# HaokunChen245/FedDAT

Hardware: AMD Instinct MI355X
Metric: VQA samples/sec, ViLT-B/32 dual-adapter local step (higher is better)
Workload: dtype fp16; 1 GPU; configs[1] with fp16 operands (BASELINE.json's configs[1] string says bf16: same operand width and MFMA rate; the bf16 step is in other_operand_format with --full): ViLT-B/32 FedDAT, 1 client per MI355X, fp16 MFMA operands (dynamic loss scale, GradScaler semantics on the device, initial 2^14), fp32 accumulate / masters, batch=32/client, 384x384 synthetic + 40-token questions, MKD on; batch_per_client=32, seq_len=185, clients=1, hip_graph=True, ranks=1, hetero_steps=False

## Files before the change

feddat_amd/albef_engine.py:

```python
from __future__ import annotations

from typing import Dict, List, Optional, Sequence

import torch

from . import lib as L
from .local_update import FlatGroup, LocalUpdateEngine, _bound

PRE = "albef_model.albef."
ADAPTER_TENSORS = ("down.weight", "down.bias", "up.weight", "up.bias")


class AlbefDatEngine(LocalUpdateEngine):
    def __init__(self, params: Dict[str, torch.Tensor], device, batch: int, n_answers: int, q_len: int = 25, a_len: int = 4,
                 vit_depth: int = 12, enc_layers: int = 12, fusion_layer: int = 6, dec_layers: int = 6, image: int = 384,
                 vocab: int = 30522, lr: float = 1e-4, weight_decay: float = 1e-2, adam_eps: float = 1e-8, pad_id: int = 0,
                 max_pos: int = 512, dropout: float = 0.0, seed: int = 0, stack_text: bool = False,
                 operands: str = "f16", loss_scale: Optional[float] = None, dynamic_loss_scale: Optional[bool] = None,
                 scale_growth_interval: int = 2000):
        self._init_loss_scale(operands, loss_scale, dynamic_loss_scale, scale_growth_interval)
        with L.operands(operands):
            self._init(params, device, batch, n_answers, q_len, a_len, vit_depth, enc_layers, fusion_layer, dec_layers, image, vocab,
                       lr, weight_decay, adam_eps, pad_id, max_pos, dropout, seed, stack_text)

# ... 256 lines not shown

    def _wgrad(self, m: int, mode: str, x, dy, rows: int):
        if mode == "both":
            n, h, g = self.ad_numel, rows // 2, self.gs["both"]
            segs = self._wgrad_desc(("wg2", m, x.data_ptr(), dy.data_ptr(), rows), lambda: [
                dict(x=x, dy=dy, z=g["z"], dz=g["dz"], grad=self.ad[0].g[m * n:(m + 1) * n], rows=h, scale=0.5),
                dict(x=x[h:], dy=dy[h:], z=g["z"][h:], dz=g["dz"][h:], grad=self.ad[1].g[m * n:(m + 1) * n], rows=h, scale=1.0)])
            ws = self.wpart_stride2
            L.adapter_wgrad_partial(segs, self.wpart["both"][m * ws:(m + 1) * ws])
            self._wg_done["both"].append(m)
            return
        a = 0 if mode == "gating" else int(mode.split("_")[1])
        if a not in self.opt_adapters:
            return
        n = self.ad_numel
        segs = self._wgrad_desc(("wg", m, a, x.data_ptr(), dy.data_ptr(), rows), lambda: [
            dict(x=x, dy=dy, z=self.gs[mode]["z"], dz=self.gs[mode]["dz"], grad=self.ad[a].g[m * n:(m + 1) * n], rows=rows,
                 scale=0.5 if mode == "gating" else 1.0)])
        ws = self.wpart_stride
        L.adapter_wgrad_partial(segs, self.wpart[mode][m * ws:(m + 1) * ws])
        self._wg_done[mode].append(m)

    def _wgrad_reduce(self, mode: str):
        done, self._wg_done[mode] = self._wg_done[mode], []
        if not done:
            return
        if mode == "both":
            ms = tuple(sorted(done))
            key = ("wg-reduce2", ms)
            if key not in self._segs_cache:
                n = self.ad_numel
                assert ms == tuple(range(ms[0], ms[0] + len(ms)))
                ptrs = [self.ad[a].g[m * n:(m + 1) * n].data_ptr() for m in ms for a in (0, 1)]
                self._segs_cache[key] = torch.tensor(ptrs, dtype=torch.int64, device=self.dev)
            ws = self.wpart_stride2
            self._reduce_wgrads(self._segs_cache[key], len(ms), 2, self.wpart["both"][ms[0] * ws:], ws, self.ovf_flags)
            return
        a = 0 if mode == "gating" else int(mode.split("_")[1])
        ms = tuple(sorted(done))
        key = ("wg-reduce", mode, ms)
        if key not in self._segs_cache:
            n, ws = self.ad_numel, self.wpart_stride
            contiguous = ms == tuple(range(ms[0], ms[0] + len(ms)))
            ptrs = torch.tensor([self.ad[a].g[m * n:(m + 1) * n].data_ptr() for m in ms], dtype=torch.int64, device=self.dev)
            self._segs_cache[key] = (ptrs, contiguous)
        ptrs, contiguous = self._segs_cache[key]
        ws, flag = self.wpart_stride, self.ovf_flags[a:a + 1]
        if contiguous:
            self._reduce_wgrads(ptrs, len(ms), 1, self.wpart[mode][ms[0] * ws:], ws, flag)
        else:
            for j, m in enumerate(ms):
                self._reduce_wgrads(ptrs[j:j + 1], 1, 1, self.wpart[mode][m * ws:], ws, flag)

    def _scale_in(self, mode: str):
        if not self._dyn():
            return dict(grad_scale=self.loss_scale)
        a = 0 if mode == "gating" else 1
        return dict(grad_scale=1.0, grad_scale_dev=self.scaler_f[0:1], nonfinite=self.ovf_flags[a:a + 1])

    _KINDS = {"emb": 0, "self_probs": 1, "self_out": 2, "cross_probs": 3, "cross_out": 4, "out": 5}

    def _drop(self, pass_id, tower: int, layer: int, kind: str):
        if pass_id is None or self.dropout <= 0:
            return None
        key = (pass_id, tower, layer, kind)
        if key not in self._segs_cache:
            k0, k1 = L.dropout_keys(self.seed, pass_id, (tower * 64 + layer) * 8 + self._KINDS[kind])
            self._segs_cache[key] = (self.dropout, k0, k1, self.drop_ctr)
        return self._segs_cache[key]

    @_bound
    def set_batch(self, batch: Dict):
        B, N, Lq, La = self.B, self.N, self.Lq, self.La
        img = batch["image"]
        if tuple(img.shape) != tuple(self.inp["image"].shape):
            raise L.FeddatHipError(f"engine built for image {tuple(self.inp['image'].shape)}, got {tuple(img.shape)}")
        self.inp["image"].copy_(img, non_blocking=True)
# ... 418 lines not shown
```

feddat_amd/csrc/adapter_wgrad.hip:

```cpp
#include "common.hip.h"

namespace {

constexpr int H = 768, R = 48, NRT = 3, CW = 64;
constexpr int NCH = H / CW;
constexpr int NBLK = 10;
constexpr int PSTRIDE = R * H + R + H;

__device__ __forceinline__ void split_bf16x2(const float (&x)[8], tbf16x8& head, tbf16x8& rest) {
    typedef unsigned int u32x4_t __attribute__((ext_vector_type(4)));
    head = cvt8_tbf16(f32x4{x[0], x[1], x[2], x[3]}, f32x4{x[4], x[5], x[6], x[7]});
    const u32x4_t hp = __builtin_bit_cast(u32x4_t, head);
    float r[8];
#pragma unroll
    for (int k = 0; k < 4; ++k) {
        r[2 * k] = x[2 * k] - __uint_as_float(hp[k] << 16);
        r[2 * k + 1] = x[2 * k + 1] - __uint_as_float(hp[k] & 0xffff0000u);
    }
    rest = cvt8_tbf16(f32x4{r[0], r[1], r[2], r[3]}, f32x4{r[4], r[5], r[6], r[7]});
}

struct WgradLaunch {
    feddat_wgrad_seg seg[2];
    float* partials;
// ... 115 lines not shown
    if (wave != 0) return;
#pragma unroll
    for (int w = 0; w < 3; ++w) {
        const float* src = red[w][lane];
#pragma unroll
        for (int rt = 0; rt < NRT; ++rt)
#pragma unroll
            for (int v = 0; v < 4; ++v) acc[rt][v] = acc[rt][v] + *reinterpret_cast<const f32x4*>(src + (rt * 4 + v) * 4);
        if (g == 0) {
            bsum = bsum + *reinterpret_cast<const f32x4*>(src + NRT * 16);
#pragma unroll
            for (int rt = 0; rt < NRT; ++rt) ssum[rt] += red_s[w][rt][i16];
        }
    }
    float* P = L.partials + ((size_t)prob * NBLK + blk) * PSTRIDE;
#pragma unroll
    for (int rt = 0; rt < NRT; ++rt)
#pragma unroll
        for (int e = 0; e < 4; ++e) {
            const int r = NRT * (4 * g + e) + rt;
            f32x4 o = {alpha * acc[rt][0][e], alpha * acc[rt][1][e], alpha * acc[rt][2][e], alpha * acc[rt][3][e]};
            *reinterpret_cast<f32x4*>(P + (size_t)r * H + c0 + 4 * i16) = o;
        }
    if (g == 0) {
        f32x4 o = {alpha * bsum[0], alpha * bsum[1], alpha * bsum[2], alpha * bsum[3]};
        *reinterpret_cast<f32x4*>(P + R * H + R + c0 + 4 * i16) = o;
        if (chunk == 0) {
#pragma unroll
            for (int rt = 0; rt < NRT; ++rt) P[R * H + NRT * i16 + rt] = unscale * ssum[rt];
        }
    }
}

__device__ __forceinline__ bool wgrad_reduce_one(const float* __restrict__ partials, float* __restrict__ gl, int seg, int i) {
    const float* Pd = partials + (size_t)(2 * seg) * NBLK * PSTRIDE;
    const float* Pu = partials + (size_t)(2 * seg + 1) * NBLK * PSTRIDE;
    float sd = 0.f, su = 0.f;
#pragma unroll 4
    for (int b = 0; b < NBLK; ++b) {
        sd += Pd[(size_t)b * PSTRIDE + i];
        su += Pu[(size_t)b * PSTRIDE + i];
    }
    if (i < R * H) {
        gl[i] = sd;
        const int r = i / H, c = i - r * H;
        gl[R * H + R + (size_t)c * R + r] = su;
        return fd_nonfinite(sd) || fd_nonfinite(su);
    }
    if (i < R * H + R) {
        gl[i] = sd;
        return fd_nonfinite(sd);
    }
    gl[R * H + R + H * R + (i - R * H - R)] = su;
    return fd_nonfinite(su);
}

__global__ __launch_bounds__(256) void wgrad_reduce_kernel(WgradLaunch L) {
    const int i = blockIdx.x * 256 + threadIdx.x;
    if (i < PSTRIDE) wgrad_reduce_one(L.partials, L.seg[blockIdx.y].grad, blockIdx.y, i);
}

struct WgradReduceBatch {
    float* const* grads;
    const float* partials;
    long stride;
    int nseg;
    int* nonfinite;
};
__global__ __launch_bounds__(256) void wgrad_reduce_batched_kernel(WgradReduceBatch B) {
    const int i = blockIdx.x * 256 + threadIdx.x;
    bool bad = false;
    if (i < PSTRIDE)
        bad = wgrad_reduce_one(B.partials + (size_t)blockIdx.z * B.stride, B.grads[blockIdx.z * B.nseg + blockIdx.y], blockIdx.y, i);
    if (B.nonfinite && __ballot(bad) != 0 && (threadIdx.x & 63) == 0) atomicOr(B.nonfinite + blockIdx.y, 1);
}

}

extern "C" long feddat_adapter_wgrad_workspace_elems(int nseg) { return (long)nseg * 2 * NBLK * PSTRIDE; }

static int wgrad_launch(const feddat_wgrad_seg* segs, int nseg, float* partials, long partials_elems, int Hd, int r,
                        bool reduce_now, hipStream_t stream) {
    FD_CHECK_ARG(segs && nseg >= 1 && nseg <= 2 && partials && Hd == H && r == R);
    FD_CHECK_ARG(partials_elems >= (long)nseg * 2 * NBLK * PSTRIDE);
    WgradLaunch L;
    L.nseg = nseg;
    L.partials = partials;
    for (int s = 0; s < nseg; ++s) {
        FD_CHECK_ARG(segs[s].x && segs[s].dy && segs[s].z && segs[s].dz && segs[s].grad && segs[s].rows > 0);
        L.seg[s] = segs[s];
    }
    if (nseg == 1) L.seg[1] = L.seg[0];
    hipLaunchKernelGGL(wgrad_kernel, dim3(NBLK, NCH, 2 * nseg), dim3(256), 0, stream, L);
    if (reduce_now) hipLaunchKernelGGL(wgrad_reduce_kernel, dim3((PSTRIDE + 255) / 256, nseg), dim3(256), 0, stream, L);
    FD_LAUNCH_RET();
}

extern "C" int feddat_adapter_wgrad(const feddat_wgrad_seg* segs, int nseg, float* partials, long partials_elems,
                                    int Hd, int r, hipStream_t stream) {
    return wgrad_launch(segs, nseg, partials, partials_elems, Hd, r, true, stream);
}

extern "C" int feddat_adapter_wgrad_partial(const feddat_wgrad_seg* segs, int nseg, float* partials, long partials_elems,
                                            int Hd, int r, hipStream_t stream) {
    return wgrad_launch(segs, nseg, partials, partials_elems, Hd, r, false, stream);
}

extern "C" int feddat_adapter_wgrad_reduce(float* const* grads_dev, int n, int nseg, const float* partials,
                                           long partials_stride, hipStream_t stream) {
    FD_CHECK_ARG(grads_dev && partials && n > 0 && n <= 65535 && nseg >= 1 && nseg <= 2);
    FD_CHECK_ARG(partials_stride >= (long)nseg * 2 * NBLK * PSTRIDE);
    hipLaunchKernelGGL(wgrad_reduce_batched_kernel, dim3((PSTRIDE + 255) / 256, nseg, n), dim3(256), 0, stream,
                       WgradReduceBatch{grads_dev, partials, partials_stride, nseg, nullptr});
    FD_LAUNCH_RET();
}

extern "C" int feddat_adapter_wgrad_reduce_checked(float* const* grads_dev, int n, int nseg, const float* partials,
                                                   long partials_stride, int* nonfinite, hipStream_t stream) {
    FD_CHECK_ARG(grads_dev && partials && n > 0 && n <= 65535 && nseg >= 1 && nseg <= 2 && nonfinite);
    FD_CHECK_ARG(partials_stride >= (long)nseg * 2 * NBLK * PSTRIDE);
    hipLaunchKernelGGL(wgrad_reduce_batched_kernel, dim3((PSTRIDE + 255) / 256, nseg, n), dim3(256), 0, stream,
                       WgradReduceBatch{grads_dev, partials, partials_stride, nseg, nonfinite});
    FD_LAUNCH_RET();
}
```

feddat_amd/csrc/head_tail.hip:

```cpp
#include "common.hip.h"

namespace {

constexpr int HT_JT = 4;
constexpr int HT_NW = 8;
constexpr int HT_U = 3;

struct HtJob {
    const float* A; long sa_i, sa_k;
    const float* B; long sb_k, sb_j;
    int I, J, K;
    int mode;
    float alpha;
    const float* alpha_dev;
    const float* bias_j;
    float* out; long ldo;
    float* colsum;
    int pro;
    const float* pro_a;
    const float* pro_b;
    float pro_eps;
    float* stats_out;
    int epi;
    const float* aux; long ld_aux;
// ... 546 lines not shown
        const float l_bce = bce / (float)B;
        scalars[0] = l_bce;
        if (nonfinite && fd_nonfinite(l_bce)) atomicOr(nonfinite, 1);
    }
}

__global__ __launch_bounds__(1024) void bce_loss_kernel(const float* __restrict__ logits, const float* __restrict__ target,
                                                        int B, int C, float* __restrict__ dlogits,
                                                        float* __restrict__ scalars, int* __restrict__ nonfinite) {
    bce_loss_body(logits, target, B, C, dlogits, scalars, nonfinite);
}

__global__ __launch_bounds__(1024) void bce_loss_rows_kernel(const float* __restrict__ logits, const float* __restrict__ target,
                                                             int n, int B, int C, float* __restrict__ dlogits,
                                                             float* __restrict__ scalars, int* __restrict__ nonfinite) {
    loss_zero_tail_rows(dlogits, n, B, C);
    bce_loss_body(logits, target, n, C, dlogits, scalars, nonfinite);
}

__device__ __forceinline__ float ht_poly_lambda(int t, int warmup, int total) {
    if (t < warmup) return (float)t / (float)max(1, warmup);
    if (t > total) return 0.f;
    return 1.0f - (float)(t - warmup) / (float)(total - warmup);
}

struct AdamwMulti {
    feddat_adamw_group grp[FEDDAT_ADAMW_MAX_GROUPS];
    int block_end[FEDDAT_ADAMW_MAX_GROUPS];
    int ngroups;
    float base_lr, beta1, beta2, eps;
    int warmup, total;
};

__global__ __launch_bounds__(256) void adamw_multi_kernel(const AdamwMulti a) {
    int k = 0;
    while (k + 1 < a.ngroups && (int)blockIdx.x >= a.block_end[k]) ++k;
    const feddat_adamw_group& G = a.grp[k];
    const int blk = (int)blockIdx.x - (k ? a.block_end[k - 1] : 0);
    const long i = ((long)blk * 256 + threadIdx.x) * 4;
    if (i >= G.n) return;
    if (G.bak_mode == 2 && G.restore_if && *G.restore_if) {
        *reinterpret_cast<f32x4*>(G.p + i) = *reinterpret_cast<const f32x4*>(G.bak + i);
        *reinterpret_cast<f32x4*>(G.m + i) = *reinterpret_cast<const f32x4*>(G.bak + G.n + i);
        *reinterpret_cast<f32x4*>(G.v + i) = *reinterpret_cast<const f32x4*>(G.bak + 2 * G.n + i);
        return;
    }
    const bool skip = (G.skip_if[0] && *G.skip_if[0]) || (G.skip_if[1] && *G.skip_if[1]);
    if (skip && G.bak_mode != 1) return;
    const int sched_t = G.state[0] + G.d_sched;
    const int t = G.state[1] + G.d_adam + 1;
    const float lr = a.base_lr * ht_poly_lambda(sched_t, a.warmup, a.total);
    int lo = 0, hi = G.nseg - 1;
    while (lo < hi) {
        const int mid = (lo + hi + 1) >> 1;
        if (G.seg_off[mid] <= i) lo = mid; else hi = mid - 1;
    }
    float wd[4];
#pragma unroll
    for (int e = 0; e < 4; ++e) wd[e] = G.seg_wd[lo];
    if (lo + 1 < G.nseg && G.seg_off[lo + 1] < i + 4) {
        for (int e = 1; e < 4; ++e) {
            int s2 = lo;
            while (s2 + 1 < G.nseg && G.seg_off[s2 + 1] <= i + e) ++s2;
            wd[e] = G.seg_wd[s2];
        }
    }
    const float bc1 = 1.0f - powf(a.beta1, (float)t);
    const float bc2 = 1.0f - powf(a.beta2, (float)t);
    f32x4 gi = *reinterpret_cast<const f32x4*>(G.g + i);
    f32x4 pi = *reinterpret_cast<const f32x4*>(G.p + i);
    f32x4 mi = *reinterpret_cast<const f32x4*>(G.m + i);
    f32x4 vi = *reinterpret_cast<const f32x4*>(G.v + i);
    if (G.bak_mode == 1) {
        *reinterpret_cast<f32x4*>(G.bak + i) = pi;
        *reinterpret_cast<f32x4*>(G.bak + G.n + i) = mi;
        *reinterpret_cast<f32x4*>(G.bak + 2 * G.n + i) = vi;
        if (skip) return;
    }
#pragma unroll
    for (int e = 0; e < 4; ++e) {
        pi[e] = pi[e] * (1.0f - lr * wd[e]);
        mi[e] = mi[e] + (gi[e] - mi[e]) * (1.0f - a.beta1);
        vi[e] = vi[e] * a.beta2 + (1.0f - a.beta2) * gi[e] * gi[e];
        const float denom = sqrtf(vi[e]) / sqrtf(bc2) + a.eps;
        pi[e] -= (lr / bc1) * (mi[e] / denom);
    }
    *reinterpret_cast<f32x4*>(G.p + i) = pi;
    *reinterpret_cast<f32x4*>(G.m + i) = mi;
    *reinterpret_cast<f32x4*>(G.v + i) = vi;
}

struct TickMulti {
    int* state[FEDDAT_ADAMW_MAX_GROUPS];
    int d_sched[FEDDAT_ADAMW_MAX_GROUPS], d_adam[FEDDAT_ADAMW_MAX_GROUPS];
    int n;
};
__global__ void step_tick_multi_kernel(const TickMulti t) {
    const int k = threadIdx.x;
    if (blockIdx.x == 0 && k < t.n) {
        t.state[k][0] += t.d_sched[k];
        t.state[k][1] += t.d_adam[k];
    }
}

__global__ void dat_step_finish_kernel(int* head_state, int* ad1_state, int* ad0_state, int* flags, float* scaler_f,
                                       int* scaler_i, float growth, float backoff, int growth_interval) {
    if (blockIdx.x != 0 || threadIdx.x != 0) return;
    const int fB = flags[0], fA = flags[1];
    const int applied = fA ? 0 : fB ? 1 : 2;
    head_state[0] += applied;
    head_state[1] += applied;
    ad1_state[0] += applied;
    ad1_state[1] += applied >= 1 ? 1 : 0;
    ad0_state[0] += applied;
    ad0_state[1] += applied == 2 ? 1 : 0;
    if (applied < 2) {
        scaler_i[1] += 2 - applied;
        scaler_i[2] += 1;
// ... 246 lines not shown
```

feddat_amd/csrc/layernorm.hip:

```cpp
#include "common.hip.h"

namespace {


template <int MAXC>
__global__ __launch_bounds__(256) void ln_fwd_kernel(const float* __restrict__ x, long x_stride,
                                                     const float* __restrict__ gamma, const float* __restrict__ beta,
                                                     float eps, int rows, int H, bf16* __restrict__ y16,
                                                     float* __restrict__ y32, float* __restrict__ stats,
                                                     unsigned char* __restrict__ y8 = nullptr,
                                                     float* __restrict__ y8_scale = nullptr) {
    const int row = blockIdx.x * 4 + (threadIdx.x >> 6);
    const int lane = threadIdx.x & 63;
    if (row >= rows) return;
    const int nc = H >> 2;
    const float* xr = x + (size_t)row * x_stride;
    f32x4 v[MAXC];
    float s = 0.f;
#pragma unroll
    for (int c = 0; c < MAXC; ++c) {
        const int i = lane + c * 64;
        if (i < nc) {
            v[c] = *reinterpret_cast<const f32x4*>(xr + i * 4);
            s += v[c][0] + v[c][1] + v[c][2] + v[c][3];
// ... 102 lines not shown
            for (int e = 0; e < 4; ++e) o[e] = rstd * (gg[c][e] - m1 - xh[c][e] * m2);
            if (dres && (dres_every == 0 || row % dres_every == 0)) {
                const size_t rr = dres_every ? (size_t)(row / dres_every) : (size_t)row;
                const f32x4 r4 = *reinterpret_cast<const f32x4*>(dres + rr * dres_stride + i * 4);
                o = o + r4;
            }
            if (out32) *reinterpret_cast<f32x4*>(out32 + (size_t)row * out_stride + i * 4) = o;
            if (out16) *reinterpret_cast<bf16x4*>(out16 + (size_t)row * H + i * 4) = cvt4(o);
            gg[c] = o;
        }
    }
    if (!out8) return;
    float amax = 0.f;
#pragma unroll
    for (int c = 0; c < MAXC; ++c)
        if (lane + c * 64 < nc)
#pragma unroll
            for (int e = 0; e < 4; ++e) amax = fmaxf(amax, fabsf(gg[c][e]));
    amax = wave_max(amax);
    const float sc = amax > 0.f ? amax * (1.0f / 448.0f) : 1.0f;
    const float inv = 1.0f / sc;
    if (lane == 0) out8_scale[row] = sc;
#pragma unroll
    for (int c = 0; c < MAXC; ++c) {
        const int i = lane + c * 64;
        if (i < nc) {
            int pk = __builtin_amdgcn_cvt_pk_fp8_f32(gg[c][0] * inv, gg[c][1] * inv, 0, false);
            pk = __builtin_amdgcn_cvt_pk_fp8_f32(gg[c][2] * inv, gg[c][3] * inv, pk, true);
            *reinterpret_cast<int*>(out8 + (size_t)row * H + i * 4) = pk;
        }
    }
}

__global__ __launch_bounds__(256) void ln_bwd_affine_kernel(const float* __restrict__ dy, const float* __restrict__ x,
                                                            const float* __restrict__ stats, int rows, int H,
                                                            float* __restrict__ dgamma, float* __restrict__ dbeta) {
    __shared__ float sg[4][64], sb[4][64];
    const int col = blockIdx.x * 64 + (threadIdx.x & 63);
    const int part = threadIdx.x >> 6;
    float ag = 0.f, ab = 0.f;
    if (col < H) {
        for (int r = part; r < rows; r += 4) {
            const float d = dy[(size_t)r * H + col];
            const float xh = (x[(size_t)r * H + col] - stats[2 * r]) * stats[2 * r + 1];
            ag += d * xh;
            ab += d;
        }
    }
    sg[part][threadIdx.x & 63] = ag;
    sb[part][threadIdx.x & 63] = ab;
    __syncthreads();
    if (part == 0 && col < H) {
        const int l = threadIdx.x;
        dgamma[col] = (sg[0][l] + sg[1][l]) + (sg[2][l] + sg[3][l]);
        dbeta[col] = (sb[0][l] + sb[1][l]) + (sb[2][l] + sb[3][l]);
    }
}

}

extern "C" int feddat_layernorm_fwd(const float* x, long x_stride, const float* gamma, const float* beta, float eps,
                                    int rows, int H, void* y_bf16, float* y_f32, float* stats, hipStream_t stream) {
    FD_CHECK_ARG(x && gamma && beta && rows > 0 && H > 0 && H % 4 == 0 && H <= 2048 && x_stride % 4 == 0);
    FD_CHECK_ARG(y_bf16 || y_f32);
#define LN_FWD(MC)                                                                                              \
    hipLaunchKernelGGL(ln_fwd_kernel<MC>, dim3((rows + 3) / 4), dim3(256), 0, stream, x, x_stride, gamma, beta, eps, \
                       rows, H, (bf16*)y_bf16, y_f32, stats)
    if (H <= 768) LN_FWD(3); else if (H <= 1536) LN_FWD(6); else LN_FWD(8);
#undef LN_FWD
    FD_LAUNCH_RET();
}

extern "C" int feddat_layernorm_fwd_fp8(const float* x, long x_stride, const float* gamma, const float* beta, float eps,
                                        int rows, int H, void* y_fp8, float* y_scale, void* y_bf16, float* stats,
                                        hipStream_t stream) {
    FD_CHECK_ARG(x && gamma && beta && rows > 0 && H > 0 && H % 4 == 0 && H <= 2048 && x_stride % 4 == 0);
    FD_CHECK_ARG(y_fp8 && y_scale);
#define LN_FWD8(MC)                                                                                              \
    hipLaunchKernelGGL(ln_fwd_kernel<MC>, dim3((rows + 3) / 4), dim3(256), 0, stream, x, x_stride, gamma, beta, eps, \
                       rows, H, (bf16*)y_bf16, (float*)nullptr, stats, (unsigned char*)y_fp8, y_scale)
    if (H <= 768) LN_FWD8(3); else if (H <= 1536) LN_FWD8(6); else LN_FWD8(8);
#undef LN_FWD8
    FD_LAUNCH_RET();
}

namespace {
__global__ __launch_bounds__(256) void quant_rows_fp8_kernel(const float* __restrict__ x, long ld, int cols,
                                                             unsigned char* __restrict__ y, float* __restrict__ scale) {
    __shared__ float red[4];
    const int row = blockIdx.x, tid = threadIdx.x;
    const float* xr = x + (size_t)row * ld;
    float amax = 0.f;
    for (int c = tid * 4; c < cols; c += 1024) {
        const f32x4 v = *reinterpret_cast<const f32x4*>(xr + c);
        amax = fmaxf(fmaxf(amax, fmaxf(fabsf(v[0]), fabsf(v[1]))), fmaxf(fabsf(v[2]), fabsf(v[3])));
    }
    amax = wave_max(amax);
    if ((tid & 63) == 0) red[tid >> 6] = amax;
    __syncthreads();
    amax = fmaxf(fmaxf(red[0], red[1]), fmaxf(red[2], red[3]));
    const float sc = amax > 0.f ? amax * (1.0f / 448.0f) : 1.0f;
    const float inv = 1.0f / sc;
    if (tid == 0) scale[row] = sc;
    for (int c = tid * 4; c < cols; c += 1024) {
        const f32x4 v = *reinterpret_cast<const f32x4*>(xr + c);
        int pk = __builtin_amdgcn_cvt_pk_fp8_f32(v[0] * inv, v[1] * inv, 0, false);
        pk = __builtin_amdgcn_cvt_pk_fp8_f32(v[2] * inv, v[3] * inv, pk, true);
        *reinterpret_cast<int*>(y + (size_t)row * cols + c) = pk;
    }
}
}

extern "C" int feddat_quant_rows_fp8(const float* x, long ld, int rows, int cols, void* y_fp8, float* scale,
                                     hipStream_t stream) {
    FD_CHECK_ARG(x && y_fp8 && scale && rows > 0 && cols > 0 && cols % 4 == 0 && ld % 4 == 0 && ld >= cols);
    hipLaunchKernelGGL(quant_rows_fp8_kernel, dim3(rows), dim3(256), 0, stream, x, ld, cols, (unsigned char*)y_fp8, scale);
    FD_LAUNCH_RET();
}

extern "C" int feddat_layernorm_bwd_dx(const void* dy_bf16, const float* dy_f32, long dy_stride, const float* x,
                                       long x_stride, const float* stats, const float* gamma, const float* dres,
                                       long dres_stride, int rows, int H, float* out_f32, long out_stride,
                                       void* out_bf16, hipStream_t stream) {
    FD_CHECK_ARG((dy_bf16 != nullptr) != (dy_f32 != nullptr));
    FD_CHECK_ARG(x && stats && gamma && rows > 0 && H > 0 && H % 4 == 0 && H <= 2048);
    FD_CHECK_ARG(dy_stride % 4 == 0 && x_stride % 4 == 0 && (!dres || dres_stride % 4 == 0));
    FD_CHECK_ARG((out_f32 && out_stride % 4 == 0) || out_bf16);
#define LN_BWD(MC)                                                                                                \
    hipLaunchKernelGGL(ln_bwd_dx_kernel<MC>, dim3((rows + 3) / 4), dim3(256), 0, stream, (const bf16*)dy_bf16, dy_f32, \
                       dy_stride, x, x_stride, stats, gamma, dres, dres_stride, rows, H, out_f32, out_stride,          \
                       (bf16*)out_bf16)
    if (H <= 768) LN_BWD(3); else if (H <= 1536) LN_BWD(6); else LN_BWD(8);
#undef LN_BWD
    FD_LAUNCH_RET();
}

extern "C" int feddat_layernorm_bwd_dx_sparse(const void* dy_bf16, const float* dy_f32, long dy_stride, const float* x,
                                              long x_stride, const float* stats, const float* gamma, const float* dres,
                                              long dres_stride, int dres_every, int rows, int H, float* out_f32,
                                              long out_stride, void* out_bf16, hipStream_t stream) {
    FD_CHECK_ARG((dy_bf16 != nullptr) != (dy_f32 != nullptr));
    FD_CHECK_ARG(x && stats && gamma && dres && dres_every > 0 && rows > 0 && H > 0 && H % 4 == 0 && H <= 2048);
    FD_CHECK_ARG(dy_stride % 4 == 0 && x_stride % 4 == 0 && dres_stride % 4 == 0);
    FD_CHECK_ARG((out_f32 && out_stride % 4 == 0) || out_bf16);
#define LN_BWDS(MC)                                                                                               \
    hipLaunchKernelGGL(ln_bwd_dx_kernel<MC>, dim3((rows + 3) / 4), dim3(256), 0, stream, (const bf16*)dy_bf16, dy_f32, \
                       dy_stride, x, x_stride, stats, gamma, dres, dres_stride, rows, H, out_f32, out_stride,          \
                       (bf16*)out_bf16, (unsigned char*)nullptr, (float*)nullptr, dres_every)
    if (H <= 768) LN_BWDS(3); else if (H <= 1536) LN_BWDS(6); else LN_BWDS(8);
#undef LN_BWDS
    FD_LAUNCH_RET();
}

extern "C" int feddat_layernorm_bwd_dx_fp8(const void* dy_bf16, const float* dy_f32, long dy_stride, const float* x,
                                           long x_stride, const float* stats, const float* gamma, const float* dres,
                                           long dres_stride, int rows, int H, float* out_f32, long out_stride,
                                           void* out_bf16, void* out_fp8, float* out_scale, hipStream_t stream) {
    FD_CHECK_ARG((dy_bf16 != nullptr) != (dy_f32 != nullptr));
    FD_CHECK_ARG(x && stats && gamma && rows > 0 && H > 0 && H % 4 == 0 && H <= 2048 && out_fp8 && out_scale);
    FD_CHECK_ARG(dy_stride % 4 == 0 && x_stride % 4 == 0 && (!dres || dres_stride % 4 == 0) && (!out_f32 || out_stride % 4 == 0));
#define LN_BWD8(MC)                                                                                               \
    hipLaunchKernelGGL(ln_bwd_dx_kernel<MC>, dim3((rows + 3) / 4), dim3(256), 0, stream, (const bf16*)dy_bf16, dy_f32, \
                       dy_stride, x, x_stride, stats, gamma, dres, dres_stride, rows, H, out_f32, out_stride,          \
                       (bf16*)out_bf16, (unsigned char*)out_fp8, out_scale)
    if (H <= 768) LN_BWD8(3); else if (H <= 1536) LN_BWD8(6); else LN_BWD8(8);
#undef LN_BWD8
    FD_LAUNCH_RET();
}

extern "C" int feddat_layernorm_bwd_full(const float* dy, const float* x, const float* stats, const float* gamma,
                                         int rows, int H, float* dx, float* dgamma, float* dbeta,
                                         hipStream_t stream) {
    FD_CHECK_ARG(dy && x && stats && gamma && dx && dgamma && dbeta && rows > 0 && rows <= 1024);
    FD_CHECK_ARG(H > 0 && H % 4 == 0 && H <= 2048);
    hipLaunchKernelGGL(ln_bwd_affine_kernel, dim3((H + 63) / 64), dim3(256), 0, stream, dy, x, stats, rows, H, dgamma,
                       dbeta);
    return feddat_layernorm_bwd_dx(nullptr, dy, (long)H, x, (long)H, stats, gamma, nullptr, 0L, rows, H, dx, (long)H,
                                   nullptr, stream);
}
```

feddat_amd/engine.py:

```python
from __future__ import annotations

from typing import Dict, Optional, Sequence, Tuple

import torch

from . import lib as L
from .local_update import FlatGroup, _bound
from .vilt_backbone import ENC, HEAD_TENSORS, ViltBackbone

ADAPTER_TENSORS = ("down.weight", "down.bias", "up.weight", "up.bias")


class ViltDatEngine(ViltBackbone):
    NPASS = 2
    ADAPTER_STEMS = ("adapter_0_", "adapter_1_", "adapter_2_")
    FFN2_STEM = "output.layer.dense."

    def __init__(self, params: Dict[str, torch.Tensor], tasks: Sequence[str], device, batch: int, res: int,
                 text_len: int = 40, layers: int = 12, num_labels: int = 100, lr: float = 1e-4,
                 weight_decay: float = 1e-2, adam_eps: float = 1e-8, wgrad_splits: int = 16, fp8: bool = False,
                 fp8_ffn_chain: bool = True, gelu_codes: bool = True, operands: Optional[str] = None,
                 loss_scale: Optional[float] = None, fp8_mx_dqkv: bool = True, dynamic_loss_scale: Optional[bool] = None,
                 scale_growth_interval: int = 2000):
        operands = operands or ("bf16" if fp8 else "f16")
# ... 357 lines not shown
            W.ln_eps = self.ln_eps
            nxt = self.act[i + 1] if i + 1 < self.nl else None
            A = L._fill(L.ViltLayerActs, h_in=a["h_in"], st1=a["st1"], qkv=a["qkv"], ctx=a["ctx"], lse=a["lse"], h2=a["h2"],
                        st2=a["st2"], u=a["u"], h3=a["h3"], z_save=self.zsave[i], h_out=nxt["h_in"] if nxt else self.h_out,
                        x16=self.x16[:R2], f16=self.f16[:R2], st1_next=nxt["st1"] if nxt else None)
            self._layer_structs[i] = (W, A, None)
        return self._layer_structs[i]

    def _grad_struct(self, cur, oth):
        key = ("G", cur.data_ptr())
        if key not in self._layer_structs:
            self._layer_structs[key] = L._fill(L.ViltLayerGrads, dh_out=cur, dh_in=oth, dh3=oth, dh16=self.dh16, dU=self.dU,
                                               dx16=self.dx16, dctx=self.dctx, dqkv=self.dqkv, z=self.z, dz=self.dz)
        return self._layer_structs[key]

    def _wgrad_segs(self, layer: int, x, x_delta_s: int, dy):
        R, n = self.R, self.ad_layer_numel
        return self._wgrad_desc(("wg", layer, x.data_ptr(), dy.data_ptr(), self.opt_adapters), lambda: [
            dict(x=x[xrow0:], dy=dy[row0:], z=self.z[row0:], dz=self.dz[row0:], grad=self.ad[a].g[layer * n:(layer + 1) * n],
                 rows=R, scale=sc)
            for a, row0, xrow0, sc in ((0, 0, 0, 0.5), (1, R, R + x_delta_s, 1.0)) if a in self.opt_adapters])

    def _wpart(self, layer: int):
        return self.wpart_all[layer * self.wpart_stride:(layer + 1) * self.wpart_stride]

    def _wgrad_reduce_all(self):
        ads = [a for a in (0, 1) if a in self.opt_adapters]
        if not ads:
            return
        key = ("wg-reduce", self.opt_adapters)
        if key not in self._segs_cache:
            n = self.ad_layer_numel
            ptrs = [self.ad[a].g[i * n:(i + 1) * n].data_ptr() for i in range(self.nl) for a in ads]
            self._segs_cache[key] = torch.tensor(ptrs, dtype=torch.int64, device=self.dev)
        self._reduce_wgrads(self._segs_cache[key], self.nl, len(ads), self.wpart_all, self.wpart_stride, self.ovf_flags[ads[0]:])

    def _adapter_wgrads(self, layer: int, x, x_delta_s: int, dy):
        segs = self._wgrad_segs(layer, x, x_delta_s, dy)
        if segs is not None:
            L.adapter_wgrad_partial(segs, self._wpart(layer))

    @_bound
    def begin_local_update(self, task: str, steps_per_epoch: int, num_epochs: int = 15, warmup_ratio: float = 0.1,
                           opt_adapters: Sequence[int] = (0, 1)):
        self.task = task
        self.copy_global_to_teacher()
        self.opt_adapters = tuple(opt_adapters)
        self._start_local_update(steps_per_epoch, num_epochs, warmup_ratio, {"adapter_0": (1, 0)})

    def _graph_switches(self) -> Tuple:
        return super()._graph_switches() + (self.use_layer_calls, self.fp8, self.fp8_ffn_chain, self.fp8_mx_dqkv, self.top_q_cls)

    def _named_groups(self):
        return [("adapter_0", self.ad[0]), ("adapter_1", self.ad[1]), ("head", self.head[self.task])]

    def _loss(self, logits, teacher, slot):
        if self.C > 128:
            flag = (self.ovf_flags[1:2] if slot == "p1" else self.ovf_flags[0:1]) if self._dyn() else None
            L.dat_loss_fwd_bwd_wide(logits, teacher, self.inp["target"], self.dlogits, self.loss_buf[slot], self.loss_ws,
                                    n=self.n_valid, nonfinite=flag)
        elif self.n_valid < self.B:
            flag = self.ovf_flags[1:2] if slot == "p1" else self.ovf_flags[0:1]
            L.dat_loss_fwd_bwd_rows(logits, teacher, self.inp["target"], self.dlogits, self.loss_buf[slot], self.n_valid,
                                    flag if self._dyn() else None)
        elif self._dyn():
            flag = self.ovf_flags[1:2] if slot == "p1" else self.ovf_flags[0:1]
# ... 64 lines not shown
```

Baseline: 4770 samples/s.

## Vectorize adapter wgrad reduce, cache AdamW segment table in LDS, persistent LayerNorm kernels

The adapter wgrad reduction now processes float4 quads. The up-projection transpose goes through an LDS tile so both the partial reads and the transposed writes are coalesced and vectorized, with alignment checks added on the host side. AdamW loads its segment/weight-decay table and bias corrections into shared memory once per block, and uses explicit FMAs. LayerNorm forward and backward-dx at H=768 switch to a grid-capped persistent kernel in which each wave walks rows and prefetches the next row while finishing the current one. The aim is to cut uncoalesced scalar memory traffic and launch/tail overhead in these small bandwidth-bound kernels, at the cost of more register pressure and code paths.

```diff
diff --git a/feddat_amd/albef_engine.py b/feddat_amd/albef_engine.py
--- a/feddat_amd/albef_engine.py
+++ b/feddat_amd/albef_engine.py
@@ -312,6 +312,7 @@
                 n = self.ad_numel
                 assert ms == tuple(range(ms[0], ms[0] + len(ms)))
                 ptrs = [self.ad[a].g[m * n:(m + 1) * n].data_ptr() for m in ms for a in (0, 1)]
+                assert all(p % 16 == 0 for p in ptrs)
                 self._segs_cache[key] = torch.tensor(ptrs, dtype=torch.int64, device=self.dev)
             ws = self.wpart_stride2
             self._reduce_wgrads(self._segs_cache[key], len(ms), 2, self.wpart["both"][ms[0] * ws:], ws, self.ovf_flags)
@@ -322,7 +323,9 @@
         if key not in self._segs_cache:
             n, ws = self.ad_numel, self.wpart_stride
             contiguous = ms == tuple(range(ms[0], ms[0] + len(ms)))
-            ptrs = torch.tensor([self.ad[a].g[m * n:(m + 1) * n].data_ptr() for m in ms], dtype=torch.int64, device=self.dev)
+            ptrs = [self.ad[a].g[m * n:(m + 1) * n].data_ptr() for m in ms]
+            assert all(p % 16 == 0 for p in ptrs)
+            ptrs = torch.tensor(ptrs, dtype=torch.int64, device=self.dev)
             self._segs_cache[key] = (ptrs, contiguous)
         ptrs, contiguous = self._segs_cache[key]
         ws, flag = self.wpart_stride, self.ovf_flags[a:a + 1]
diff --git a/feddat_amd/csrc/adapter_wgrad.hip b/feddat_amd/csrc/adapter_wgrad.hip
--- a/feddat_amd/csrc/adapter_wgrad.hip
+++ b/feddat_amd/csrc/adapter_wgrad.hip
@@ -171,32 +171,58 @@
     }
 }
 
-__device__ __forceinline__ bool wgrad_reduce_one(const float* __restrict__ partials, float* __restrict__ gl, int seg, int i) {
+constexpr int RED_T = 384, RED_UC = 32;
+constexpr int RED_UT = H / RED_UC;
+constexpr int RED_DQ = (R * H + R) / 4;
+constexpr int RED_DB = (RED_DQ + RED_T - 1) / RED_T;
+constexpr int RED_BLOCKS = RED_UT + RED_DB + 1;
+constexpr int RED_LD = R + 4;
+static_assert(R * RED_UC == 4 * RED_T && H % RED_UC == 0 && (R * H) % 4 == 0 && R % 4 == 0 && H / 4 <= RED_T, "reduce tiling");
+
+__device__ __forceinline__ f32x4 wgrad_sum_partials(const float* __restrict__ p0) {
+    f32x4 p[NBLK];
+#pragma unroll
+    for (int b = 0; b < NBLK; ++b) p[b] = *reinterpret_cast<const f32x4*>(p0 + (size_t)b * PSTRIDE);
+    f32x4 s = {0.f, 0.f, 0.f, 0.f};
+#pragma unroll
+    for (int b = 0; b < NBLK; ++b) s = s + p[b];
+    return s;
+}
+__device__ __forceinline__ bool fd_nonfinite4(const f32x4 v) {
+    return fd_nonfinite(v[0]) || fd_nonfinite(v[1]) || fd_nonfinite(v[2]) || fd_nonfinite(v[3]);
+}
+
+__device__ __forceinline__ bool wgrad_reduce_block(const float* __restrict__ partials, float* __restrict__ gl, int seg) {
+    __shared__ __attribute__((aligned(16))) float tile[RED_UC * RED_LD];
     const float* Pd = partials + (size_t)(2 * seg) * NBLK * PSTRIDE;
     const float* Pu = partials + (size_t)(2 * seg + 1) * NBLK * PSTRIDE;
-    float sd = 0.f, su = 0.f;
-#pragma unroll 4
-    for (int b = 0; b < NBLK; ++b) {
-        sd += Pd[(size_t)b * PSTRIDE + i];
-        su += Pu[(size_t)b * PSTRIDE + i];
-    }
-    if (i < R * H) {
-        gl[i] = sd;
-        const int r = i / H, c = i - r * H;
-        gl[R * H + R + (size_t)c * R + r] = su;
-        return fd_nonfinite(sd) || fd_nonfinite(su);
-    }
-    if (i < R * H + R) {
-        gl[i] = sd;
-        return fd_nonfinite(sd);
-    }
-    gl[R * H + R + H * R + (i - R * H - R)] = su;
-    return fd_nonfinite(su);
-}
-
-__global__ __launch_bounds__(256) void wgrad_reduce_kernel(WgradLaunch L) {
-    const int i = blockIdx.x * 256 + threadIdx.x;
-    if (i < PSTRIDE) wgrad_reduce_one(L.partials, L.seg[blockIdx.y].grad, blockIdx.y, i);
+    const int blk = blockIdx.x, q = threadIdx.x;
+    if (blk < RED_UT) {
+        const int c0 = blk * RED_UC, r = q / (RED_UC / 4), cq = q % (RED_UC / 4);
+        const f32x4 su = wgrad_sum_partials(Pu + (size_t)r * H + c0 + 4 * cq);
+#pragma unroll
+        for (int e = 0; e < 4; ++e) tile[(4 * cq + e) * RED_LD + r] = su[e];
+        __syncthreads();
+        const int c = q / (R / 4), r4 = 4 * (q % (R / 4));
+        const f32x4 o = *reinterpret_cast<const f32x4*>(tile + c * RED_LD + r4);
+        *reinterpret_cast<f32x4*>(gl + R * H + R + (size_t)(c0 + c) * R + r4) = o;
+        return fd_nonfinite4(o);
+    }
+    if (blk < RED_UT + RED_DB) {
+        const int i = ((blk - RED_UT) * RED_T + q) * 4;
+        if (i >= R * H + R) return false;
+        const f32x4 sd = wgrad_sum_partials(Pd + i);
+        *reinterpret_cast<f32x4*>(gl + i) = sd;
+        return fd_nonfinite4(sd);
+    }
+    if (q >= H / 4) return false;
+    const f32x4 su = wgrad_sum_partials(Pu + R * H + R + 4 * q);
+    *reinterpret_cast<f32x4*>(gl + R * H + R + H * R + 4 * q) = su;
+    return fd_nonfinite4(su);
+}
+
+__global__ __launch_bounds__(RED_T) void wgrad_reduce_kernel(WgradLaunch L) {
+    wgrad_reduce_block(L.partials, L.seg[blockIdx.y].grad, blockIdx.y);
 }
 
 struct WgradReduceBatch {
@@ -206,11 +232,9 @@
     int nseg;
     int* nonfinite;
 };
-__global__ __launch_bounds__(256) void wgrad_reduce_batched_kernel(WgradReduceBatch B) {
-    const int i = blockIdx.x * 256 + threadIdx.x;
-    bool bad = false;
-    if (i < PSTRIDE)
-        bad = wgrad_reduce_one(B.partials + (size_t)blockIdx.z * B.stride, B.grads[blockIdx.z * B.nseg + blockIdx.y], blockIdx.y, i);
+__global__ __launch_bounds__(RED_T) void wgrad_reduce_batched_kernel(WgradReduceBatch B) {
+    const bool bad =
+        wgrad_reduce_block(B.partials + (size_t)blockIdx.z * B.stride, B.grads[blockIdx.z * B.nseg + blockIdx.y], blockIdx.y);
     if (B.nonfinite && __ballot(bad) != 0 && (threadIdx.x & 63) == 0) atomicOr(B.nonfinite + blockIdx.y, 1);
 }
 
@@ -227,11 +251,12 @@
     L.partials = partials;
     for (int s = 0; s < nseg; ++s) {
         FD_CHECK_ARG(segs[s].x && segs[s].dy && segs[s].z && segs[s].dz && segs[s].grad && segs[s].rows > 0);
+        FD_CHECK_ARG(!reduce_now || (((uintptr_t)segs[s].grad | (uintptr_t)partials) & 15) == 0);
         L.seg[s] = segs[s];
     }
     if (nseg == 1) L.seg[1] = L.seg[0];
     hipLaunchKernelGGL(wgrad_kernel, dim3(NBLK, NCH, 2 * nseg), dim3(256), 0, stream, L);
-    if (reduce_now) hipLaunchKernelGGL(wgrad_reduce_kernel, dim3((PSTRIDE + 255) / 256, nseg), dim3(256), 0, stream, L);
+    if (reduce_now) hipLaunchKernelGGL(wgrad_reduce_kernel, dim3(RED_BLOCKS, nseg), dim3(RED_T), 0, stream, L);
     FD_LAUNCH_RET();
 }
 
@@ -249,7 +274,8 @@
                                            long partials_stride, hipStream_t stream) {
     FD_CHECK_ARG(grads_dev && partials && n > 0 && n <= 65535 && nseg >= 1 && nseg <= 2);
     FD_CHECK_ARG(partials_stride >= (long)nseg * 2 * NBLK * PSTRIDE);
-    hipLaunchKernelGGL(wgrad_reduce_batched_kernel, dim3((PSTRIDE + 255) / 256, nseg, n), dim3(256), 0, stream,
+    FD_CHECK_ARG(((uintptr_t)partials & 15) == 0 && partials_stride % 4 == 0);
+    hipLaunchKernelGGL(wgrad_reduce_batched_kernel, dim3(RED_BLOCKS, nseg, n), dim3(RED_T), 0, stream,
                        WgradReduceBatch{grads_dev, partials, partials_stride, nseg, nullptr});
     FD_LAUNCH_RET();
 }
@@ -258,7 +284,8 @@
                                                    long partials_stride, int* nonfinite, hipStream_t stream) {
     FD_CHECK_ARG(grads_dev && partials && n > 0 && n <= 65535 && nseg >= 1 && nseg <= 2 && nonfinite);
     FD_CHECK_ARG(partials_stride >= (long)nseg * 2 * NBLK * PSTRIDE);
-    hipLaunchKernelGGL(wgrad_reduce_batched_kernel, dim3((PSTRIDE + 255) / 256, nseg, n), dim3(256), 0, stream,
+    FD_CHECK_ARG(((uintptr_t)partials & 15) == 0 && partials_stride % 4 == 0);
+    hipLaunchKernelGGL(wgrad_reduce_batched_kernel, dim3(RED_BLOCKS, nseg, n), dim3(RED_T), 0, stream,
                        WgradReduceBatch{grads_dev, partials, partials_stride, nseg, nonfinite});
     FD_LAUNCH_RET();
 }
diff --git a/feddat_amd/csrc/head_tail.hip b/feddat_amd/csrc/head_tail.hip
--- a/feddat_amd/csrc/head_tail.hip
+++ b/feddat_amd/csrc/head_tail.hip
@@ -602,17 +602,47 @@
     int warmup, total;
 };
 
+__device__ __forceinline__ void adamw_quad_wd(const long* off, const float* wdv, const int nseg, const long i, float (&wd)[4]) {
+    int lo = 0, hi = nseg - 1;
+    while (lo < hi) {
+        const int mid = (lo + hi + 1) >> 1;
+        if (off[mid] <= i) lo = mid; else hi = mid - 1;
+    }
+#pragma unroll
+    for (int e = 0; e < 4; ++e) wd[e] = wdv[lo];
+    if (lo + 1 < nseg && off[lo + 1] < i + 4) {
+        for (int e = 1; e < 4; ++e) {
+            int s2 = lo;
+            while (s2 + 1 < nseg && off[s2 + 1] <= i + e) ++s2;
+            wd[e] = wdv[s2];
+        }
+    }
+}
+
+constexpr int ADAMW_SEG_LDS = 1024;
 __global__ __launch_bounds__(256) void adamw_multi_kernel(const AdamwMulti a) {
+    __shared__ long s_off[ADAMW_SEG_LDS];
+    __shared__ float s_wd[ADAMW_SEG_LDS];
+    __shared__ float s_bc[2];
     int k = 0;
     while (k + 1 < a.ngroups && (int)blockIdx.x >= a.block_end[k]) ++k;
     const feddat_adamw_group& G = a.grp[k];
     const int blk = (int)blockIdx.x - (k ? a.block_end[k - 1] : 0);
     const long i = ((long)blk * 256 + threadIdx.x) * 4;
-    if (i >= G.n) return;
+    const bool live = i < G.n;
+    f32x4 gi = {0.f, 0.f, 0.f, 0.f}, pi = gi, mi = gi, vi = gi;
+    if (live) {
+        gi = *reinterpret_cast<const f32x4*>(G.g + i);
+        pi = *reinterpret_cast<const f32x4*>(G.p + i);
+        mi = *reinterpret_cast<const f32x4*>(G.m + i);
+        vi = *reinterpret_cast<const f32x4*>(G.v + i);
+    }
     if (G.bak_mode == 2 && G.restore_if && *G.restore_if) {
-        *reinterpret_cast<f32x4*>(G.p + i) = *reinterpret_cast<const f32x4*>(G.bak + i);
-        *reinterpret_cast<f32x4*>(G.m + i) = *reinterpret_cast<const f32x4*>(G.bak + G.n + i);
-        *reinterpret_cast<f32x4*>(G.v + i) = *reinterpret_cast<const f32x4*>(G.bak + 2 * G.n + i);
+        if (live) {
+            *reinterpret_cast<f32x4*>(G.p + i) = *reinterpret_cast<const f32x4*>(G.bak + i);
+            *reinterpret_cast<f32x4*>(G.m + i) = *reinterpret_cast<const f32x4*>(G.bak + G.n + i);
+            *reinterpret_cast<f32x4*>(G.v + i) = *reinterpret_cast<const f32x4*>(G.bak + 2 * G.n + i);
+        }
         return;
     }
     const bool skip = (G.skip_if[0] && *G.skip_if[0]) || (G.skip_if[1] && *G.skip_if[1]);
@@ -620,27 +650,22 @@
     const int sched_t = G.state[0] + G.d_sched;
     const int t = G.state[1] + G.d_adam + 1;
     const float lr = a.base_lr * ht_poly_lambda(sched_t, a.warmup, a.total);
-    int lo = 0, hi = G.nseg - 1;
-    while (lo < hi) {
-        const int mid = (lo + hi + 1) >> 1;
-        if (G.seg_off[mid] <= i) lo = mid; else hi = mid - 1;
-    }
+    const bool table_in_lds = G.nseg <= ADAMW_SEG_LDS;
+    if (table_in_lds)
+        for (int s = threadIdx.x; s < G.nseg; s += 256) {
+            s_off[s] = G.seg_off[s];
+            s_wd[s] = G.seg_wd[s];
+        }
+    if (threadIdx.x == 0) {
+        s_bc[0] = 1.0f - powf(a.beta1, (float)t);
+        s_bc[1] = 1.0f - powf(a.beta2, (float)t);
+    }
+    __syncthreads();
+    if (!live) return;
     float wd[4];
-#pragma unroll
-    for (int e = 0; e < 4; ++e) wd[e] = G.seg_wd[lo];
-    if (lo + 1 < G.nseg && G.seg_off[lo + 1] < i + 4) {
-        for (int e = 1; e < 4; ++e) {
-            int s2 = lo;
-            while (s2 + 1 < G.nseg && G.seg_off[s2 + 1] <= i + e) ++s2;
-            wd[e] = G.seg_wd[s2];
-        }
-    }
-    const float bc1 = 1.0f - powf(a.beta1, (float)t);
-    const float bc2 = 1.0f - powf(a.beta2, (float)t);
-    f32x4 gi = *reinterpret_cast<const f32x4*>(G.g + i);
-    f32x4 pi = *reinterpret_cast<const f32x4*>(G.p + i);
-    f32x4 mi = *reinterpret_cast<const f32x4*>(G.m + i);
-    f32x4 vi = *reinterpret_cast<const f32x4*>(G.v + i);
+    if (table_in_lds) adamw_quad_wd(s_off, s_wd, G.nseg, i, wd);
+    else adamw_quad_wd(G.seg_off, G.seg_wd, G.nseg, i, wd);
+    const float bc1 = s_bc[0], bc2 = s_bc[1];
     if (G.bak_mode == 1) {
         *reinterpret_cast<f32x4*>(G.bak + i) = pi;
         *reinterpret_cast<f32x4*>(G.bak + G.n + i) = mi;
@@ -649,11 +674,12 @@
     }
 #pragma unroll
     for (int e = 0; e < 4; ++e) {
-        pi[e] = pi[e] * (1.0f - lr * wd[e]);
-        mi[e] = mi[e] + (gi[e] - mi[e]) * (1.0f - a.beta1);
-        vi[e] = vi[e] * a.beta2 + (1.0f - a.beta2) * gi[e] * gi[e];
+#pragma clang fp contract(off)
+        const float keep = __builtin_fmaf(-lr, wd[e], 1.0f);
+        mi[e] = __builtin_fmaf(gi[e] - mi[e], 1.0f - a.beta1, mi[e]);
+        vi[e] = __builtin_fmaf(vi[e], a.beta2, (1.0f - a.beta2) * gi[e] * gi[e]);
         const float denom = sqrtf(vi[e]) / sqrtf(bc2) + a.eps;
-        pi[e] -= (lr / bc1) * (mi[e] / denom);
+        pi[e] = __builtin_fmaf(pi[e], keep, -((lr / bc1) * (mi[e] / denom)));
     }
     *reinterpret_cast<f32x4*>(G.p + i) = pi;
     *reinterpret_cast<f32x4*>(G.m + i) = mi;
diff --git a/feddat_amd/csrc/layernorm.hip b/feddat_amd/csrc/layernorm.hip
--- a/feddat_amd/csrc/layernorm.hip
+++ b/feddat_amd/csrc/layernorm.hip
@@ -158,6 +158,160 @@
     }
 }
 
+constexpr int LN_WALK_BLOCKS_PER_CU = 2;
+
+template <int MAXC>
+__global__ __launch_bounds__(256) void ln_fwd_walk_kernel(const float* __restrict__ x, long x_stride,
+                                                          const float* __restrict__ gamma, const float* __restrict__ beta,
+                                                          float eps, int rows, bf16* __restrict__ y16,
+                                                          float* __restrict__ y32, float* __restrict__ stats) {
+    constexpr int H = 256 * MAXC;
+    const int lane = threadIdx.x & 63;
+    const int nwaves = gridDim.x * 4;
+    int row = blockIdx.x * 4 + __builtin_amdgcn_readfirstlane(threadIdx.x >> 6);
+    if (row >= rows) return;
+    f32x4 g4[MAXC], b4[MAXC], va[MAXC], vb[MAXC];
+    auto load = [&](f32x4(&v)[MAXC], int r) {
+#pragma unroll
+        for (int c = 0; c < MAXC; ++c) v[c] = *reinterpret_cast<const f32x4*>(x + (size_t)r * x_stride + (lane + c * 64) * 4);
+    };
+    auto finish = [&](const f32x4(&v)[MAXC], int r) {
+#pragma clang fp contract(off)
+        float s = 0.f;
+#pragma unroll
+        for (int c = 0; c < MAXC; ++c) s += v[c][0] + v[c][1] + v[c][2] + v[c][3];
+        const float mean = wave_sum(s) / (float)H;
+        float q = 0.f;
+#pragma unroll
+        for (int c = 0; c < MAXC; ++c)
+#pragma unroll
+            for (int e = 0; e < 4; ++e) {
+                const float d = v[c][e] - mean;
+                q += d * d;
+            }
+        const float rstd = rsqrtf(wave_sum(q) / (float)H + eps);
+        if (stats && lane == 0) {
+            stats[2 * r] = mean;
+            stats[2 * r + 1] = rstd;
+        }
+#pragma unroll
+        for (int c = 0; c < MAXC; ++c) {
+            const int i = lane + c * 64;
+            f32x4 o;
+#pragma unroll
+            for (int e = 0; e < 4; ++e) o[e] = __builtin_fmaf((v[c][e] - mean) * rstd, g4[c][e], b4[c][e]);
+            if (y16) *reinterpret_cast<bf16x4*>(y16 + (size_t)r * H + i * 4) = cvt4(o);
+            if (y32) *reinterpret_cast<f32x4*>(y32 + (size_t)r * H + i * 4) = o;
+        }
+    };
+    load(va, row);
+#pragma unroll
+    for (int c = 0; c < MAXC; ++c) {
+        g4[c] = *reinterpret_cast<const f32x4*>(gamma + (lane + c * 64) * 4);
+        b4[c] = *reinterpret_cast<const f32x4*>(beta + (lane + c * 64) * 4);
+    }
+    for (;;) {
+        const int next = row + nwaves;
+        load(vb, next < rows ? next : row);
+        finish(va, row);
+        if (next >= rows) return;
+        row = next;
+        __builtin_amdgcn_sched_barrier(0);
+#pragma unroll
+        for (int c = 0; c < MAXC; ++c) va[c] = vb[c];
+    }
+}
+
+template <int MAXC, bool DY16, int DRES>
+struct LnBwdRow {
+    f32x4 x[MAXC], r[MAXC], d32[MAXC];
+    bf16x4 d16[MAXC];
+    float mean, rstd;
+    bool add_r;
+    __device__ __forceinline__ void load(const int row, const int lane, const void* dy, long dy_stride, const float* x_,
+                                         long x_stride, const float* stats, const float* dres, long dres_stride,
+                                         int dres_every) {
+        mean = stats[2 * row];
+        rstd = stats[2 * row + 1];
+        add_r = DRES == 1 || (DRES == 2 && row % dres_every == 0);
+        const size_t rr = DRES == 2 ? (size_t)(row / dres_every) : (size_t)row;
+#pragma unroll
+        for (int c = 0; c < MAXC; ++c) {
+            const int i = lane + c * 64;
+            x[c] = *reinterpret_cast<const f32x4*>(x_ + (size_t)row * x_stride + i * 4);
+            if (DY16) d16[c] = *reinterpret_cast<const bf16x4*>((const bf16*)dy + (size_t)row * dy_stride + i * 4);
+            else d32[c] = *reinterpret_cast<const f32x4*>((const float*)dy + (size_t)row * dy_stride + i * 4);
+            if (DRES) r[c] = *reinterpret_cast<const f32x4*>(dres + rr * dres_stride + i * 4);
+        }
+    }
+};
+
+template <int MAXC, bool DY16, int DRES>
+__global__ __launch_bounds__(256) void ln_bwd_dx_walk_kernel(const void* __restrict__ dy, long dy_stride,
+                                                             const float* __restrict__ x, long x_stride,
+                                                             const float* __restrict__ stats, const float* __restrict__ gamma,
+                                                             const float* __restrict__ dres, long dres_stride, int rows,
+                                                             float* __restrict__ out32, long out_stride,
+                                                             bf16* __restrict__ out16, const int dres_every) {
+    static_assert(MAXC == 3, "finish() spells out ln_bwd_dx_kernel<3>'s fused multiply-adds");
+    constexpr int H = 256 * MAXC;
+    const int lane = threadIdx.x & 63;
+    const int nwaves = gridDim.x * 4;
+    int row = blockIdx.x * 4 + __builtin_amdgcn_readfirstlane(threadIdx.x >> 6);
+    if (row >= rows) return;
+    f32x4 g4[MAXC];
+    LnBwdRow<MAXC, DY16, DRES> ra, rb;
+    auto load = [&](LnBwdRow<MAXC, DY16, DRES>& R, int r) {
+        R.load(r, lane, dy, dy_stride, x, x_stride, stats, dres, dres_stride, dres_every);
+    };
+    auto finish = [&](const LnBwdRow<MAXC, DY16, DRES>& R, int r) {
+#pragma clang fp contract(off)
+        const float mean = R.mean, rstd = R.rstd;
+        f32x4 xh[MAXC], gg[MAXC];
+        float s1 = 0.f, s2 = 0.f;
+#pragma unroll
+        for (int c = 0; c < MAXC; ++c) {
+            f32x4 d;
+            if (DY16) d = f32x4{(float)R.d16[c][0], (float)R.d16[c][1], (float)R.d16[c][2], (float)R.d16[c][3]};
+            else d = R.d32[c];
+#pragma unroll
+            for (int e = 0; e < 4; ++e) {
+                xh[c][e] = (R.x[c][e] - mean) * rstd;
+                gg[c][e] = d[e] * g4[c][e];
+                s1 += gg[c][e];
+                s2 += gg[c][e] * xh[c][e];
+            }
+        }
+        const float m1 = wave_sum(s1) / (float)H;
+        const float m2 = wave_sum(s2) / (float)H;
+#pragma unroll
+        for (int c = 0; c < MAXC; ++c) {
+            const int i = lane + c * 64;
+            f32x4 o;
+#pragma unroll
+            for (int e = 0; e < 4; ++e) {
+                const float t = gg[c][e] - m1;
+                o[e] = rstd * (c == 2 && e >= 2 ? t - xh[c][e] * m2 : __builtin_fmaf(-xh[c][e], m2, t));
+            }
+            if (DRES && R.add_r) o = o + R.r[c];
+            if (out32) *reinterpret_cast<f32x4*>(out32 + (size_t)r * out_stride + i * 4) = o;
+            if (out16) *reinterpret_cast<bf16x4*>(out16 + (size_t)r * H + i * 4) = cvt4(o);
+        }
+    };
+    load(ra, row);
+#pragma unroll
+    for (int c = 0; c < MAXC; ++c) g4[c] = *reinterpret_cast<const f32x4*>(gamma + (lane + c * 64) * 4);
+    for (;;) {
+        const int next = row + nwaves;
+        load(rb, next < rows ? next : row);
+        finish(ra, row);
+        if (next >= rows) return;
+        row = next;
+        __builtin_amdgcn_sched_barrier(0);
+        ra = rb;
+    }
+}
+
 __global__ __launch_bounds__(256) void ln_bwd_affine_kernel(const float* __restrict__ dy, const float* __restrict__ x,
                                                             const float* __restrict__ stats, int rows, int H,
                                                             float* __restrict__ dgamma, float* __restrict__ dbeta) {
@@ -185,6 +339,33 @@
 
 }
 
+static int ln_walk_grid(int rows, int* grid) {
+    int n_cu = 0;
+    if (fd_device_cus(&n_cu) != FEDDAT_OK) return FEDDAT_ELAUNCH;
+    const int need = (rows + 3) / 4, cap = n_cu * LN_WALK_BLOCKS_PER_CU;
+    *grid = need < cap ? need : cap;
+    return FEDDAT_OK;
+}
+
+static int ln_bwd_dx_walk(const void* dy_bf16, const float* dy_f32, long dy_stride, const float* x, long x_stride,
+                          const float* stats, const float* gamma, const float* dres, long dres_stride, int dres_every, int rows,
+                          float* out_f32, long out_stride, void* out_bf16, hipStream_t stream) {
+    int grid;
+    if (ln_walk_grid(rows, &grid) != FEDDAT_OK) return FEDDAT_ELAUNCH;
+    const void* dy = dy_bf16 ? dy_bf16 : (const void*)dy_f32;
+#define LN_WALK(DY16, DRES)                                                                                              \
+    hipLaunchKernelGGL((ln_bwd_dx_walk_kernel<3, DY16, DRES>), dim3(grid), dim3(256), 0, stream, dy, dy_stride, x, x_stride, \
+                       stats, gamma, dres, dres_stride, rows, out_f32, out_stride, (bf16*)out_bf16, dres_every)
+    const int mode = !dres ? 0 : dres_every ? 2 : 1;
+    if (dy_bf16) {
+        if (mode == 0) LN_WALK(true, 0); else if (mode == 1) LN_WALK(true, 1); else LN_WALK(true, 2);
+    } else {
+        if (mode == 0) LN_WALK(false, 0); else if (mode == 1) LN_WALK(false, 1); else LN_WALK(false, 2);
+    }
+#undef LN_WALK
+    FD_LAUNCH_RET();
+}
+
 extern "C" int feddat_layernorm_fwd(const float* x, long x_stride, const float* gamma, const float* beta, float eps,
                                     int rows, int H, void* y_bf16, float* y_f32, float* stats, hipStream_t stream) {
     FD_CHECK_ARG(x && gamma && beta && rows > 0 && H > 0 && H % 4 == 0 && H <= 2048 && x_stride % 4 == 0);
@@ -192,7 +373,12 @@
 #define LN_FWD(MC)                                                                                              \
     hipLaunchKernelGGL(ln_fwd_kernel<MC>, dim3((rows + 3) / 4), dim3(256), 0, stream, x, x_stride, gamma, beta, eps, \
                        rows, H, (bf16*)y_bf16, y_f32, stats)
-    if (H <= 768) LN_FWD(3); else if (H <= 1536) LN_FWD(6); else LN_FWD(8);
+    if (H == 768) {
+        int grid;
+        if (ln_walk_grid(rows, &grid) != FEDDAT_OK) return FEDDAT_ELAUNCH;
+        hipLaunchKernelGGL(ln_fwd_walk_kernel<3>, dim3(grid), dim3(256), 0, stream, x, x_stride, gamma, beta, eps, rows,
+                           (bf16*)y_bf16, y_f32, stats);
+    } else if (H <= 768) LN_FWD(3); else if (H <= 1536) LN_FWD(6); else LN_FWD(8);
 #undef LN_FWD
     FD_LAUNCH_RET();
 }
@@ -256,6 +442,9 @@
     hipLaunchKernelGGL(ln_bwd_dx_kernel<MC>, dim3((rows + 3) / 4), dim3(256), 0, stream, (const bf16*)dy_bf16, dy_f32, \
                        dy_stride, x, x_stride, stats, gamma, dres, dres_stride, rows, H, out_f32, out_stride,          \
                        (bf16*)out_bf16)
+    if (H == 768)
+        return ln_bwd_dx_walk(dy_bf16, dy_f32, dy_stride, x, x_stride, stats, gamma, dres, dres_stride, 0, rows, out_f32,
+                              out_stride, out_bf16, stream);
     if (H <= 768) LN_BWD(3); else if (H <= 1536) LN_BWD(6); else LN_BWD(8);
 #undef LN_BWD
     FD_LAUNCH_RET();
@@ -273,6 +462,9 @@
     hipLaunchKernelGGL(ln_bwd_dx_kernel<MC>, dim3((rows + 3) / 4), dim3(256), 0, stream, (const bf16*)dy_bf16, dy_f32, \
                        dy_stride, x, x_stride, stats, gamma, dres, dres_stride, rows, H, out_f32, out_stride,          \
                        (bf16*)out_bf16, (unsigned char*)nullptr, (float*)nullptr, dres_every)
+    if (H == 768)
+        return ln_bwd_dx_walk(dy_bf16, dy_f32, dy_stride, x, x_stride, stats, gamma, dres, dres_stride, dres_every, rows,
+                              out_f32, out_stride, out_bf16, stream);
     if (H <= 768) LN_BWDS(3); else if (H <= 1536) LN_BWDS(6); else LN_BWDS(8);
 #undef LN_BWDS
     FD_LAUNCH_RET();
diff --git a/feddat_amd/engine.py b/feddat_amd/engine.py
--- a/feddat_amd/engine.py
+++ b/feddat_amd/engine.py
@@ -413,6 +413,7 @@
         if key not in self._segs_cache:
             n = self.ad_layer_numel
             ptrs = [self.ad[a].g[i * n:(i + 1) * n].data_ptr() for i in range(self.nl) for a in ads]
+            assert all(p % 16 == 0 for p in ptrs)
             self._segs_cache[key] = torch.tensor(ptrs, dtype=torch.int64, device=self.dev)
         self._reduce_wgrads(self._segs_cache[key], self.nl, len(ads), self.wpart_all, self.wpart_stride, self.ovf_flags[ads[0]:])
 
```

After: 4832 samples/s, median of 6. 1.3% higher.
